# CNR-STIIMA-IRAS/rosdyn

Measured on NVIDIA B200. Metric: 6-DOF regressor+torque samples/sec (fp64), higher is better.
Workload: dtype f64

## Files before the change

### rosdyn_b200/csrc/gram_common.cuh

```cuda
#pragma once
#ifndef __CUDACC_RTC__
#include <cuda_runtime.h>
#endif

#include "chain_dev.h"
#include "spatial.cuh"

namespace rdb
{

#ifndef GF_TSPLIT
#define GF_TSPLIT 2
#endif
#ifndef GF_ZCOL
#define GF_ZCOL 1
#endif
constexpr int GF_KSPLIT = 4;
constexpr int GF_TS = GF_TSPLIT;
constexpr int GF_MMA_WARPS = GF_KSPLIT * GF_TS;
constexpr int GF_MAX_SLOTS = 4;
constexpr int GF_BAR_REDUCE = 1;

__device__ __forceinline__ void bar_sync(int id, int count) { asm volatile("bar.sync %0, %1;" ::"r"(id), "r"(count) : "memory"); }
__device__ __forceinline__ void dmma884f(double& d0, double& d1, double a, double b)
{
  asm volatile("mma.sync.aligned.m8n8k4.row.col.f64.f64.f64.f64 {%0,%1}, {%2}, {%3}, {%0,%1};\n" : "+d"(d0), "+d"(d1) : "d"(a), "d"(b));
}
__device__ __forceinline__ uint32_t smem_u32(const void* p) { return (uint32_t)__cvta_generic_to_shared(p); }
__device__ __forceinline__ void mbar_init(uint64_t* b, int count)
{
  asm volatile("mbarrier.init.shared::cta.b64 [%0], %1;" ::"r"(smem_u32(b)), "r"(count) : "memory");
}
__device__ __forceinline__ void mbar_arrive(uint64_t* b)
{
  asm volatile("{\n .reg .b64 st;\n mbarrier.arrive.shared::cta.b64 st, [%0];\n}" ::"r"(smem_u32(b)) : "memory");
}
__device__ __forceinline__ void mbar_wait(uint64_t* b, uint32_t parity)
{
  asm volatile(
      "{\n .reg .pred p;\n"
      "W: mbarrier.try_wait.parity.shared::cta.b64 p, [%0], %1;\n"
      " @p bra D;\n bra W;\n"
      "D:\n}" ::"r"(smem_u32(b)),
      "r"(parity)
      : "memory");
}

template <int V>
struct ic
{
  static constexpr int value = V;
};
template <int B, int E, class F>
__device__ __forceinline__ void static_for(F&& f)
{
  if constexpr (B < E)
  {
    f(ic<B>{});
    static_for<B + 1, E>(f);
  }
}

constexpr int GX_COLS = 8;
#ifndef GF_TAU_TILE
#define GF_TAU_TILE 0
#endif
template <int NJ, int X = 0, int Z = 0>
struct GramGeom
{
  static constexpr int P = 10 * NJ;
  static constexpr int TC = Z == 2 && !GF_TAU_TILE ? 0 : 1;
  __host__ __device__ static constexpr int inblk(int p)
  {
    constexpr int zord[10] = {9, 1, 2, 8, 3, 4, 5, 6, 7, 0};
    return Z == 2 ? zord[p] : (Z == 1 ? (p == 0 ? 9 : p - 1) : p);
  }
  __host__ __device__ static constexpr int param_at(int q)
  {
    constexpr int zinv[10] = {9, 1, 2, 4, 5, 6, 7, 8, 3, 0};
    return Z == 2 ? zinv[q] : (Z == 1 ? (q == 9 ? 0 : q + 1) : q);
  }
  __host__ __device__ static constexpr int pos(int l, int p) { return TC + 10 * (NJ - 1 - l) + inblk(p); }
  __host__ __device__ static constexpr bool stored(int j, int l, int p)
  {
    if (j != l || Z == 0) return true;
    if (Z == 1) return p != 0;
    return l == 0 ? (p == 1 || p == 2 || p == 9) : (p != 0 && p != 3);
  }
  __host__ __device__ static constexpr int rowlen(int j)
  {
    return Z == 2 ? TC + 10 * (NJ - 1 - j) + (j == 0 ? 3 : 8) : 1 + 10 * (NJ - j) - Z;
  }
  static constexpr int NPOS = rowlen(0);
  __host__ __device__ static constexpr int col_of(int q) { return q < TC ? P : 10 * (NJ - 1 - (q - TC) / 10) + param_at((q - TC) % 10); }
  __host__ __device__ static constexpr bool has_pos(int c) { return c / 10 > 0 || stored(0, 0, c % 10); }
  static constexpr int T = (NPOS + 7) / 8;
  static constexpr int NT = T * (T + 1) / 2;
  static constexpr int NF = T + 1 - TC;
  static constexpr int PARTIAL = NT * 64 + (TC ? 0 : 8 * T + 1);
  static constexpr int KPW = 8 / GF_KSPLIT;
  static constexpr int NSTEPS = NJ * KPW;
  __host__ __device__ static constexpr int threads(int slots) { return 32 * (GF_MMA_WARPS + slots); }
  __host__ __device__ static constexpr int rowbase(int j)
  {
    int o = 0;
    for (int i = 0; i < j; i++) o += (rowlen(i) + (X ? GX_COLS : 0)) * 32;
    return o;
  }
  __host__ __device__ static constexpr int taubase(int j) { return TC ? rowbase(j) : rowbase(NJ) + 32 * j; }
  static constexpr int SLOT_DOUBLES = rowbase(NJ) + (TC ? 0 : 32 * NJ);
  __host__ __device__ static constexpr int tile(int I, int J) { return I * T - I * (I - 1) / 2 + (J - I); }
  __host__ __device__ static constexpr bool owns(int I, int ts, int par) { return ts == 1 || (I & 1) == par; }
  __host__ __device__ static constexpr int ntiles(int ts, int par)
  {
    int n = 0;
    for (int I = 0; I < T; I++)
      if (owns(I, ts, par)) n += T - I;
    return n > 0 ? n : 1;
  }
  __host__ __device__ static constexpr int local(int I, int J, int ts, int par)
  {
    int n = 0;
    for (int K = 0; K < I; K++)
      if (owns(K, ts, par)) n += T - K;
    return n + (J - I);
  }
  __host__ __device__ static constexpr int bown(int I, int ts, int par)
  {
    int n = 0;
    for (int K = 0; K < I; K++)
      if (owns(K, ts, par)) n++;
    return n;
  }
  __host__ __device__ static constexpr int nbacc(int ts, int par) { return TC || (par != 0 && bown(T, ts, par) == 0) ? 1 : bown(T, ts, par) + (par == 0 ? 1 : 0); }
  __host__ __device__ static constexpr int tj(int j) { return (rowlen(j) + 7) / 8; }
  __host__ __device__ static constexpr int xtile(int j, int I)
  {
    int n = 0;
    for (int k = 0; k < j; k++) n += tj(k) + 1;
    return n + I;
  }
  __host__ __device__ static constexpr int nxt()
  {
    int n = 0;
    for (int k = 0; k < NJ; k++) n += tj(k) + 1;
    return n;
  }
  static constexpr int NXT = nxt();
  __host__ __device__ static constexpr bool xowns(int j, int I, int ts, int par) { return ts == 1 || ((I == tj(j) ? j : I) & 1) == par; }
  __host__ __device__ static constexpr int xlocal(int j, int I, int ts, int par)
  {
    int n = 0;
    for (int k = 0; k <= j; k++)
      for (int K = 0; K <= tj(k); K++)
      {
        if (k == j && K == I) return n;
        if (xowns(k, K, ts, par)) n++;
      }
    return n;
  }
  __host__ __device__ static constexpr int nxtiles(int ts, int par)
  {
    int n = 0;
    for (int k = 0; k < NJ; k++)
      for (int K = 0; K <= tj(k); K++)
        if (xowns(k, K, ts, par)) n++;
    return n;
  }
};

enum : int
{
  GXK_SAT = 1,
  GXK_OMEGA = 2,
  GXK_SGN = 3,
  GXK_SQ = 4,
  GXK_Q = 5,
  GXK_ONE = 6
};
struct GramComps
{
  int32_t ncols[8];
  int32_t kind[8][GX_COLS];
  double thr[8][GX_COLS], vmax[8][GX_COLS];
  double ithr[8][GX_COLS];
};

struct RtModel
{
  static constexpr bool RUNTIME = true;
};
enum : int
{
  MK_A = 0,
  MK_T = 1,
  MK_PI = 2,
  MK_G = 3
};
struct Zr
{
};
template <int S>
struct Un
{
};
template <class T>
struct tv_unit
{
  static constexpr int s = 0;
};
template <int S>
struct tv_unit<Un<S>>
{
  static constexpr int s = S;
};
template <class T>
struct tv_zero
{
  static constexpr bool v = false;
};
template <>
struct tv_zero<Zr>
{
  static constexpr bool v = true;
};

template <class M, int F, int L, int K, int NJ>
__device__ __forceinline__ auto kc(const ChainDev<NJ>& C)
{
  if constexpr (M::RUNTIME)
  {
    if constexpr (F == MK_A) return C.joint[L].A[K];
    else if constexpr (F == MK_T) return C.joint[L].t[K];
    else if constexpr (F == MK_PI) return C.link[L].pi[K];
    else return C.g[K];
  }
  else
  {
    constexpr double v = M::val(F, L, K);
    if constexpr (v == 0.0) return Zr{};
    else if constexpr (v == 1.0) return Un<1>{};
    else if constexpr (v == -1.0) return Un<-1>{};
    else return v;
  }
}

template <class A>
__device__ __forceinline__ double tv_d(A a)
{
  if constexpr (tv_zero<A>::v) return 0.0;
  else if constexpr (tv_unit<A>::s != 0) return (double)tv_unit<A>::s;
  else return a;
}
template <class A>
__device__ __forceinline__ auto tneg(A a)
{
  if constexpr (tv_zero<A>::v) return Zr{};
  else if constexpr (tv_unit<A>::s != 0) return Un<-tv_unit<A>::s>{};
  else return -a;
}
template <class A, class B>
__device__ __forceinline__ auto tmul(A a, B b)
{
  constexpr int ua = tv_unit<A>::s, ub = tv_unit<B>::s;
  if constexpr (tv_zero<A>::v || tv_zero<B>::v) return Zr{};
  else if constexpr (ua != 0 && ub != 0) return Un<ua * ub>{};
  else if constexpr (ua != 0) return ua > 0 ? b : -b;
  else if constexpr (ub != 0) return ub > 0 ? a : -a;
  else return __dmul_rn(a, b);
}
template <class A, class B>
__device__ __forceinline__ auto tadd(A a, B b)
{
  if constexpr (tv_zero<A>::v) return b;
  else if constexpr (tv_zero<B>::v) return a;
  else return __dadd_rn(tv_d(a), tv_d(b));
}
template <class A, class B, class C>
__device__ __forceinline__ auto tfma(A a, B b, C c)
{
  using P = decltype(tmul(a, b));
  if constexpr (tv_zero<P>::v) return c;
  else if constexpr (tv_zero<C>::v) return tmul(a, b);
  else if constexpr (tv_unit<A>::s != 0 || tv_unit<B>::s != 0) return tadd(tmul(a, b), c);
  else return __fma_rn(a, b, tv_d(c));
}

template <class X, class Y, class W>
struct T3
{
  X x;
  Y y;
  W z;
};
template <class X, class Y, class W>
__device__ __forceinline__ T3<X, Y, W> mk3(X x, Y y, W z)
{
  return T3<X, Y, W>{x, y, z};
}
template <class A>
__device__ __forceinline__ V3 tod3(const A& a)
{
  return V3{tv_d(a.x), tv_d(a.y), tv_d(a.z)};
}
template <class A, class B>
__device__ __forceinline__ auto tdot(const A& a, const B& b)
{
  return tfma(a.x, b.x, tfma(a.y, b.y, tmul(a.z, b.z)));
}
template <class A, class B>
__device__ __forceinline__ auto tcross(const A& a, const B& b)
{
  return mk3(tfma(a.y, b.z, tneg(tmul(a.z, b.y))), tfma(a.z, b.x, tneg(tmul(a.x, b.z))), tfma(a.x, b.y, tneg(tmul(a.y, b.x))));
}
template <class Cv, class A, class B>
__device__ __forceinline__ auto tcross_add(const Cv& c, const A& a, const B& b)
{
  return mk3(tfma(a.y, b.z, tfma(tneg(a.z), b.y, c.x)), tfma(a.z, b.x, tfma(tneg(a.x), b.z, c.y)), tfma(a.x, b.y, tfma(tneg(a.y), b.x, c.z)));
}
template <class R, class A>
__device__ __forceinline__ auto trotT(const R& r, const A& a)
{
  return mk3(tfma(r.x.x, a.x, tfma(r.y.x, a.y, tmul(r.z.x, a.z))), tfma(r.x.y, a.x, tfma(r.y.y, a.y, tmul(r.z.y, a.z))),
             tfma(r.x.z, a.x, tfma(r.y.z, a.y, tmul(r.z.z, a.z))));
}

template <int NJ>
struct GenIn
{
  double q[NJ], dq[NJ], ddq[NJ], sv[NJ], cv[NJ];
};
template <int NJ>
__device__ __forceinline__ void gen_load(const ChainDev<NJ>& C, const SamplesDev& in, int64_t i, GenIn<NJ>& x)
{
#pragma unroll
  for (int l = 0; l < NJ; l++)
  {
    x.q[l] = ld_in(in.q, C.joint[l].in, in.ld, i);
    x.dq[l] = ld_in(in.dq, C.joint[l].in, in.ld, i);
    x.ddq[l] = ld_in(in.ddq, C.joint[l].in, in.ld, i);
  }
}

template <int NJ>
__device__ __forceinline__ void gram_component_columns(const ChainDev<NJ>& C, const GramComps& comps, const SamplesDev& in, int64_t i,
                                                       double* __restrict__ slot, int lane)
{
  using G = GramGeom<NJ, 1>;
  double qv[NJ], dqv[NJ];
#pragma unroll
  for (int j = 0; j < NJ; j++)
  {
    qv[j] = ld_in(in.q, C.joint[j].in, in.ld, i);
    dqv[j] = ld_in(in.dq, C.joint[j].in, in.ld, i);
  }
  static_for<0, NJ>([&](auto jc) {
    constexpr int j = decltype(jc)::value;
    const double q = qv[j], dq = dqv[j];
    const int nc = comps.ncols[j];
    double* o = slot + G::rowbase(j) + G::rowlen(j) * 32;
#pragma unroll 1
    for (int c = 0; c < GX_COLS; c++)
    {
      double val = 0.0;
      if (c < nc)
      {
        const int kd = comps.kind[j][c];
        const double th = comps.thr[j][c], vm = comps.vmax[j][c];
        const double omega = fmin(fmax(dq, -vm), vm);
        if (kd == GXK_OMEGA) val = omega;
        else if (kd == GXK_Q) val = q;
        else if (kd == GXK_ONE) val = 1.0;
        else
        {
          const double r = omega * comps.ithr[j][c];
          if (kd == GXK_SAT) val = fmin(fmax(r, -1.0), 1.0);
          else
          {
            const double sg = omega == 0.0 ? 0.0 : (omega > th ? 1.0 : (omega < -th ? -1.0 : r));
            val = kd == GXK_SGN ? sg : omega * omega * sg;
          }
        }
      }
      o[c * 32 + (lane ^ (4 * (c & 3)))] = val;
    }
  });
}

template <bool GLOBAL>
__device__ __forceinline__ void st_row(double* p, double v)
{
  if (GLOBAL) __stcg(p, v);
  else *p = v;
}

template <class M, int NJ, int X, int Z, bool GLOBAL, int L, int J, bool OWN, class E0, class E1, class E2, class E3, class E4, class E5, class E6,
          class E7, class E8, class E9>
__device__ __forceinline__ void gram_emit(const ChainDev<NJ>& C, double (&tau)[NJ], double* __restrict__ slot, int lane, E0 e0, E1 e1, E2 e2, E3 e3,
                                          E4 e4, E5 e5, E6 e6, E7 e7, E8 e8, E9 e9)
{
  using G = GramGeom<NJ, X, Z>;
  auto P = [&](auto pc) { return kc<M, MK_PI, L, decltype(pc)::value>(C); };
  auto t0a = [&] {
    if constexpr (J == L && M::RUNTIME) return 0.0;
    else if constexpr (J == L) return Zr{};
    else return tau[J];
  }();
  const auto t0 = tfma(e8, P(ic<8>{}), tfma(e6, P(ic<6>{}), tfma(e4, P(ic<4>{}), tfma(e2, P(ic<2>{}), tfma(e0, P(ic<0>{}), t0a)))));
  const auto t1 = tfma(e9, P(ic<9>{}), tfma(e7, P(ic<7>{}), tfma(e5, P(ic<5>{}), tfma(e3, P(ic<3>{}), tmul(e1, P(ic<1>{}))))));
  tau[J] = tv_d(tadd(t0, t1));
  double* o = slot + G::rowbase(J);
  const double e[10] = {tv_d(e0), tv_d(e1), tv_d(e2), tv_d(e3), tv_d(e4), tv_d(e5), tv_d(e6), tv_d(e7), tv_d(e8), tv_d(e9)};
#pragma unroll
  for (int p = 0; p < 10; p++)
    if (G::stored(J, L, p))
      st_row<GLOBAL>(o + G::pos(L, p) * 32 + (lane ^ (4 * (G::pos(L, p) & 3))), e[p]);
}
template <class M, int NJ, int X, int Z, bool GLOBAL, int L, int J, class U, class S>
__device__ __forceinline__ void gram_project(const ChainDev<NJ>& C, double (&tau)[NJ], double* __restrict__ slot, int lane, const U& u, const S& s,
                                             const V3& fm, const V3& w, const V3& al)
{
  const auto h = tcross_add(tcross_add(tcross(u, al), w, tcross(w, u)), fm, s);
  const auto rho = tcross(s, w);
  gram_emit<M, NJ, X, Z, GLOBAL, L, J, false>(
      C, tau, slot, lane, tdot(u, fm), h.x, h.y, h.z, tfma(s.x, al.x, tmul(rho.x, w.x)),
      tfma(s.x, al.y, tfma(s.y, al.x, tfma(rho.x, w.y, tmul(rho.y, w.x)))), tfma(s.x, al.z, tfma(s.z, al.x, tfma(rho.x, w.z, tmul(rho.z, w.x)))),
      tfma(s.y, al.y, tmul(rho.y, w.y)), tfma(s.y, al.z, tfma(s.z, al.y, tfma(rho.y, w.z, tmul(rho.z, w.y)))), tfma(s.z, al.z, tmul(rho.z, w.z)));
}

template <int NJ, class M, int X, int Z, bool GLOBAL, bool LAZY>
__device__ __forceinline__ void gram_walk_rev(const ChainDev<NJ>& C, const GenIn<NJ>& x, const SamplesDev& in, double* __restrict__ slot, int64_t i,
                                              int lane, double (&tau)[NJ])
{
  static_assert(REV_AXIS[0] == 0.0 && REV_AXIS[1] == 0.0 && REV_AXIS[2] == 1.0, "the REV walk below is written for the axis s = e_z");
  V3 U[NJ], S[NJ];
  V3 v = v3(0, 0, 0), w = v3(0, 0, 0), a = v3(0, 0, 0), al = v3(0, 0, 0), g;
  static_for<0, NJ>([&](auto lc) {
    constexpr int l = decltype(lc)::value;
    const JointDev& J = C.joint[l];
    const double dql = LAZY ? ld_in(in.dq, J.in, in.ld, i) : x.dq[l], ddql = LAZY ? ld_in(in.ddq, J.in, in.ld, i) : x.ddq[l];
    const double sl = x.sv[l], cl = x.cv[l];
    const auto t = mk3(kc<M, MK_T, l, 0>(C), kc<M, MK_T, l, 1>(C), kc<M, MK_T, l, 2>(C));
    auto row = [&](auto kc_) {
      constexpr int k = decltype(kc_)::value;
      const auto a0 = kc<M, MK_A, l, 3 * k>(C);
      const auto a1 = kc<M, MK_A, l, 3 * k + 1>(C);
      return mk3(tfma(sl, a1, tmul(cl, a0)), tfma(-sl, a0, tmul(cl, a1)), kc<M, MK_A, l, 3 * k + 2>(C));
    };
    const auto R = mk3(row(ic<0>{}), row(ic<1>{}), row(ic<2>{}));
    v = tod3(trotT(R, tcross_add(v, w, t)));
    w = tod3(trotT(R, w));
    a = tod3(trotT(R, tcross_add(a, al, t)));
    al = tod3(trotT(R, al));
    if constexpr (l == 0) g = tod3(trotT(R, mk3(kc<M, MK_G, 0, 0>(C), kc<M, MK_G, 0, 1>(C), kc<M, MK_G, 0, 2>(C))));
    else g = tod3(trotT(R, g));
    w.z += dql;
    a.x = fma(v.y, dql, a.x);
    a.y = fma(-v.x, dql, a.y);
    al.x = fma(w.y, dql, al.x);
    al.y = fma(-w.x, dql, al.y);
    al.z += ddql;
    static_for<0, (l > 0 ? l - 1 : 0)>([&](auto jc) {
      constexpr int j = decltype(jc)::value;
      U[j] = tod3(trotT(R, tcross_add(U[j], S[j], t)));
      S[j] = tod3(trotT(R, S[j]));
    });
    const auto S1 = R.z;
    const auto U1 = mk3(tfma(t.x, R.y.x, tneg(tmul(t.y, R.x.x))), tfma(t.x, R.y.y, tneg(tmul(t.y, R.x.y))), tfma(t.x, R.y.z, tneg(tmul(t.y, R.x.z))));
    if constexpr (l > 0)
    {
      S[l - 1] = tod3(S1);
      U[l - 1] = tod3(U1);
    }
    const V3 fm = cross_add(a - g, w, v);
    static_for<0, l + 1>([&](auto jc) {
      constexpr int j = decltype(jc)::value;
      if constexpr (j == l)
      {
        const double e7 = w.x * w.y;
        gram_emit<M, NJ, X, Z, GLOBAL, l, j, true>(C, tau, slot, lane, Zr{}, fm.y, -fm.x, Zr{}, -e7, fma(w.x, w.x, -(w.y * w.y)),
                                                   fma(-w.y, w.z, al.x), e7, fma(w.x, w.z, al.y), al.z);
      }
      else if constexpr (j == l - 1) gram_project<M, NJ, X, Z, GLOBAL, l, j>(C, tau, slot, lane, U1, S1, fm, w, al);
      else gram_project<M, NJ, X, Z, GLOBAL, l, j>(C, tau, slot, lane, U[j], S[j], fm, w, al);
    });
  });
}

template <int NJ, int X, int Z, bool GLOBAL, bool LAZY>
__device__ __forceinline__ void gram_walk_gen(const ChainDev<NJ>& C, const GenIn<NJ>& x, const SamplesDev& in, double* __restrict__ slot, int64_t i,
                                              int lane, double (&tau)[NJ])
{
  using G = GramGeom<NJ, X, Z>;
  V3 U[NJ], S[NJ];
  V3 v = v3(0, 0, 0), w = v3(0, 0, 0), a = v3(0, 0, 0), al = v3(0, 0, 0);
  V3 g = v3(C.g);
#pragma unroll
  for (int l = 0; l < NJ; l++)
  {
    const JointDev& J = C.joint[l];
    const double dql = LAZY ? ld_in(in.dq, J.in, in.ld, i) : x.dq[l], ddql = LAZY ? ld_in(in.ddq, J.in, in.ld, i) : x.ddq[l];
    double R[9];
    const V3 t = J.type != RDB_JOINT_PRISMATIC ? v3(J.t) : axpy(v3(J.t), v3(J.axp), x.q[l]);
    if (J.type == RDB_JOINT_REVOLUTE)
    {
      const double c1 = 1.0 - x.cv[l];
#pragma unroll
      for (int k = 0; k < 9; k++) R[k] = fma(c1, J.C[k], fma(x.sv[l], J.B[k], J.A[k]));
    }
    else
    {
#pragma unroll
      for (int k = 0; k < 9; k++) R[k] = J.A[k];
    }
    v = rotT(R, cross_add(v, w, t));
    w = rotT(R, w);
    a = rotT(R, cross_add(a, al, t));
    al = rotT(R, al);
    g = rotT(R, g);
    const V3 axj = v3(J.ax);
    const V3 su = J.type == RDB_JOINT_PRISMATIC ? axj : v3(0, 0, 0);
    const V3 ss = J.type == RDB_JOINT_REVOLUTE ? axj : v3(0, 0, 0);
    v = axpy(v, su, dql);
    w = axpy(w, ss, dql);
    const V3 xl = cross_add(cross(w, su), v, ss);
    const V3 xa = cross(w, ss);
    a = axpy(axpy(a, xl, dql), su, ddql);
    al = axpy(axpy(al, xa, dql), ss, ddql);
    U[l] = su;
    S[l] = ss;
#pragma unroll
    for (int j = 0; j < l; j++)
    {
      U[j] = rotT(R, cross_add(U[j], S[j], t));
      S[j] = rotT(R, S[j]);
    }
    tau[l] = 0.0;
    const double* Pl = C.link[l].pi;
    const V3 fm = cross_add(a - g, w, v);
#pragma unroll
    for (int j = 0; j <= l; j++)
    {
      const V3 u = U[j], s = S[j];
      const V3 h = cross_add(cross_add(cross(u, al), w, cross(w, u)), fm, s);
      const V3 rho = cross(s, w);
      double e[10];
      e[0] = dot(u, fm);
      e[1] = h.x;
      e[2] = h.y;
      e[3] = h.z;
      e[4] = fma(s.x, al.x, rho.x * w.x);
      e[5] = fma(s.x, al.y, fma(s.y, al.x, fma(rho.x, w.y, rho.y * w.x)));
      e[6] = fma(s.x, al.z, fma(s.z, al.x, fma(rho.x, w.z, rho.z * w.x)));
      e[7] = fma(s.y, al.y, rho.y * w.y);
      e[8] = fma(s.y, al.z, fma(s.z, al.y, fma(rho.y, w.z, rho.z * w.y)));
      e[9] = fma(s.z, al.z, rho.z * w.z);
      double t0 = tau[j], t1 = e[1] * Pl[1];
#pragma unroll
      for (int p = 0; p < 10; p += 2) t0 = fma(e[p], Pl[p], t0);
#pragma unroll
      for (int p = 3; p < 10; p += 2) t1 = fma(e[p], Pl[p], t1);
      tau[j] = t0 + t1;
      double* o = slot + G::rowbase(j);
#pragma unroll
      for (int p = 0; p < 10; p++) st_row<GLOBAL>(o + G::pos(l, p) * 32 + (lane ^ (4 * (G::pos(l, p) & 3))), e[p]);
    }
  }
}

template <int NJ, bool REV, int X, int Z = 0, bool GLOBAL = false, bool LAZY = false, class M = RtModel>
__device__ __forceinline__ void gram_generate(const ChainDev<NJ>& C, const GramComps* comps, const GenIn<NJ>& x, const SamplesDev& in,
                                              const double* __restrict__ tau_meas, double* __restrict__ slot, int64_t i, int lane)
{
  static_assert(!Z || REV, "the zero mass column of a link on its own joint exists for revolute joints only");
  static_assert(REV || M::RUNTIME, "compile-time models are built for the REV walk");
  using G = GramGeom<NJ, X, Z>;
  double tau[NJ];
  if constexpr (REV) gram_walk_rev<NJ, M, X, Z, GLOBAL, LAZY>(C, x, in, slot, i, lane, tau);
  else gram_walk_gen<NJ, X, Z, GLOBAL, LAZY>(C, x, in, slot, i, lane, tau);
#pragma unroll
  for (int j = 0; j < NJ; j++)
  {
    const double tv = tau_meas ? __ldcs(tau_meas + (int64_t)C.joint[j].in * in.ld + i) : tau[j];
    st_row<GLOBAL>(slot + G::taubase(j) + lane, tv);
  }
  if (X) gram_component_columns<NJ>(C, *comps, in, i, slot, lane);
}

template <int NJ, int X, int Z = 0, bool GLOBAL = false>
__device__ __noinline__ void gram_zero_lane(double* __restrict__ slot, int lane)
{
  using G = GramGeom<NJ, X, Z>;
  for (int j = 0; j < NJ; j++)
  {
    for (int c = 0; c < G::rowlen(j); c++) st_row<GLOBAL>(slot + G::rowbase(j) + c * 32 + (lane ^ (4 * (c & 3))), 0.0);
    if (!G::TC) st_row<GLOBAL>(slot + G::taubase(j) + lane, 0.0);
    if (X)
      for (int c = 0; c < GX_COLS; c++) st_row<GLOBAL>(slot + G::rowbase(j) + (G::rowlen(j) + c) * 32 + (lane ^ (4 * (c & 3))), 0.0);
  }
}

}
```

### rosdyn_b200/csrc/gram_fused.cuh

```cuda
#pragma once
#include "gram_common.cuh"

namespace rdb
{

template <int NJ, int J, int X = 0, int Z = 0>
__device__ __forceinline__ void gram_load_frags(const double* __restrict__ slot, int kk, int lane, double (&b)[GramGeom<NJ, 0, Z>::NF])
{
  using G = GramGeom<NJ, X, Z>;
  constexpr int T = G::T, L = G::rowlen(J), TJ = G::tj(J);
  const int g = lane >> 2, t = lane & 3;
  const double* rowp = slot + G::rowbase(J) + ((4 * kk + t) ^ (4 * (g & 3)));
#pragma unroll
  for (int I = 0; I < T; I++)
  {
    if (I >= TJ) continue;
    const int col = 8 * I + g;
    if (8 * I + 7 < L || col < L) b[I] = rowp[col * 32];
    else b[I] = 0.0;
  }
  if constexpr (!G::TC) b[T] = slot[G::taubase(J) + 4 * kk + t];
}
template <int NJ, int PAR, int J, int Z>
__device__ __forceinline__ void gram_mma_step(const double (&b)[GramGeom<NJ, 0, Z>::NF], double (&acc)[GramGeom<NJ, 0, Z>::ntiles(GF_TS, PAR)][2])
{
  using G = GramGeom<NJ, 0, Z>;
  constexpr int T = G::T, TJ = G::tj(J);
#pragma unroll
  for (int I = 0; I < T; I++)
  {
    if (I >= TJ || !G::owns(I, GF_TS, PAR)) continue;
#pragma unroll
    for (int K = I; K < T; K++)
      if (K < TJ) dmma884f(acc[G::local(I, K, GF_TS, PAR)][0], acc[G::local(I, K, GF_TS, PAR)][1], b[I], b[K]);
  }
}
template <int NJ, int PAR, int J, int Z>
__device__ __forceinline__ void gram_tau_step(const double (&b)[GramGeom<NJ, 0, Z>::NF], double (&bacc)[GramGeom<NJ, 0, Z>::nbacc(GF_TS, PAR)])
{
  using G = GramGeom<NJ, 0, Z>;
  if constexpr (!G::TC)
  {
    static_for<0, G::tj(J)>([&](auto Ic) {
      constexpr int I = decltype(Ic)::value;
      if constexpr (G::owns(I, GF_TS, PAR)) bacc[G::bown(I, GF_TS, PAR)] = fma(b[I], b[G::T], bacc[G::bown(I, GF_TS, PAR)]);
    });
    if constexpr (PAR == 0) bacc[G::nbacc(GF_TS, PAR) - 1] = fma(b[G::T], b[G::T], bacc[G::nbacc(GF_TS, PAR) - 1]);
  }
}
template <int NJ, int PAR, int STEP, int Z>
__device__ __forceinline__ void gram_consume_steps(const double* __restrict__ slot, int ks, int lane, const double (&bcur)[GramGeom<NJ, 0, Z>::NF],
                                                   double (&acc)[GramGeom<NJ, 0, Z>::ntiles(GF_TS, PAR)][2],
                                                   double (&bacc)[GramGeom<NJ, 0, Z>::nbacc(GF_TS, PAR)])
{
  using G = GramGeom<NJ, 0, Z>;
  constexpr int J = STEP / G::KPW;
  if constexpr (STEP + 1 < G::NSTEPS)
  {
    double bnext[G::NF];
    gram_load_frags<NJ, (STEP + 1) / G::KPW, 0, Z>(slot, ks * G::KPW + (STEP + 1) % G::KPW, lane, bnext);
    gram_mma_step<NJ, PAR, J, Z>(bcur, acc);
    gram_tau_step<NJ, PAR, J, Z>(bcur, bacc);
    gram_consume_steps<NJ, PAR, STEP + 1, Z>(slot, ks, lane, bnext, acc, bacc);
  }
  else
  {
    gram_mma_step<NJ, PAR, J, Z>(bcur, acc);
    gram_tau_step<NJ, PAR, J, Z>(bcur, bacc);
  }
}
template <int NJ, int PAR, int Z>
__device__ __forceinline__ void gram_consume_slot(const double* __restrict__ slot, int ks, int lane,
                                                  double (&acc)[GramGeom<NJ, 0, Z>::ntiles(GF_TS, PAR)][2],
                                                  double (&bacc)[GramGeom<NJ, 0, Z>::nbacc(GF_TS, PAR)])
{
  using G = GramGeom<NJ, 0, Z>;
  double b0[G::NF];
  gram_load_frags<NJ, 0, 0, Z>(slot, ks * G::KPW, lane, b0);
  gram_consume_steps<NJ, PAR, 0, Z>(slot, ks, lane, b0, acc, bacc);
}

#ifndef GF_SPIN_NS
#define GF_SPIN_NS 32
#endif
struct GramBars
{
  uint64_t full[GF_MAX_SLOTS], empty[GF_MAX_SLOTS];
  uint32_t filled[GF_MAX_SLOTS];
  uint32_t drained[GF_MAX_SLOTS];
};
__device__ __forceinline__ uint32_t ld_acquire_u32(const uint32_t* p)
{
  uint32_t v;
  asm volatile("ld.acquire.cta.shared.u32 %0, [%1];" : "=r"(v) : "r"(smem_u32(p)) : "memory");
  return v;
}
__device__ __forceinline__ void st_release_u32(uint32_t* p, uint32_t v)
{
  asm volatile("st.release.cta.shared.u32 [%0], %1;" ::"r"(smem_u32(p)), "r"(v) : "memory");
}
__device__ __forceinline__ void red_release_inc(uint32_t* p)
{
  asm volatile("red.release.cta.shared.add.u32 [%0], 1;" ::"r"(smem_u32(p)) : "memory");
}
__device__ __forceinline__ void wait_counter_ge(const uint32_t* p, uint32_t v)
{
  while (ld_acquire_u32(p) < v) __nanosleep(GF_SPIN_NS);
}

template <int NJ, int PAR, int Z>
__device__ __forceinline__ void gram_mma_reduce(double (&acc)[GramGeom<NJ, 0, Z>::ntiles(GF_TS, PAR)][2], double* smem, int ks, int lane)
{
  using G = GramGeom<NJ, 0, Z>;
  bar_sync(GF_BAR_REDUCE, 32 * GF_MMA_WARPS);
  const int g = lane >> 2, t = lane & 3;
  for (int w = 0; w < GF_KSPLIT; w++)
  {
    if (ks == w)
    {
#pragma unroll
      for (int I = 0; I < G::T; I++)
      {
        if (!G::owns(I, GF_TS, PAR)) continue;
#pragma unroll
        for (int J = I; J < G::T; J++)
        {
          double* o = smem + G::tile(I, J) * 64 + g * 8 + 2 * t;
          const int k = G::local(I, J, GF_TS, PAR);
          if (w == 0)
          {
            o[0] = acc[k][0];
            o[1] = acc[k][1];
          }
          else
          {
            o[0] += acc[k][0];
            o[1] += acc[k][1];
          }
        }
      }
    }
    bar_sync(GF_BAR_REDUCE, 32 * GF_MMA_WARPS);
  }
}
template <int NJ, int PAR, int Z>
__device__ __forceinline__ void gram_tau_reduce(double (&bacc)[GramGeom<NJ, 0, Z>::nbacc(GF_TS, PAR)], double* smem, int ks, int lane)
{
  using G = GramGeom<NJ, 0, Z>;
  if constexpr (!G::TC)
  {
    constexpr int NB = G::nbacc(GF_TS, PAR);
#pragma unroll
    for (int k = 0; k < NB; k++)
    {
      bacc[k] += __shfl_xor_sync(0xffffffffu, bacc[k], 1);
      bacc[k] += __shfl_xor_sync(0xffffffffu, bacc[k], 2);
    }
    const int g = lane >> 2, t = lane & 3;
    double* ob = smem + G::NT * 64;
    for (int w = 0; w < GF_KSPLIT; w++)
    {
      if (ks == w && t == 0)
      {
#pragma unroll
        for (int I = 0; I < G::T; I++)
        {
          if (!G::owns(I, GF_TS, PAR)) continue;
          double& o = ob[8 * I + g];
          o = w == 0 ? bacc[G::bown(I, GF_TS, PAR)] : o + bacc[G::bown(I, GF_TS, PAR)];
        }
        if (PAR == 0 && g == 0) ob[8 * G::T] = w == 0 ? bacc[NB - 1] : ob[8 * G::T] + bacc[NB - 1];
      }
      bar_sync(GF_BAR_REDUCE, 32 * GF_MMA_WARPS);
    }
  }
}

template <int NJ, int SLOTS, int PAR, int Z>
__device__ __forceinline__ void gram_mma_role(const SamplesDev& in, double* smem, GramBars* bars, int ks, int lane, int dbg)
{
  using G = GramGeom<NJ, 0, Z>;
  constexpr int NTP = G::ntiles(GF_TS, PAR);
  double acc[NTP][2], bacc[G::nbacc(GF_TS, PAR)];
#pragma unroll
  for (int k = 0; k < NTP; k++) acc[k][0] = acc[k][1] = 0.0;
#pragma unroll
  for (int k = 0; k < G::nbacc(GF_TS, PAR); k++) bacc[k] = 0.0;
  const int64_t ngroups = (in.n + 31) / 32;
  const int64_t stride = (int64_t)gridDim.x * SLOTS;
  uint32_t parity = 0;
  for (int64_t base = (int64_t)blockIdx.x * SLOTS; base < ngroups; base += stride, parity ^= 1)
  {
#pragma unroll 1
    for (int s = 0; s < SLOTS; s++)
    {
      if (base + s >= ngroups) break;
      const double* slot = smem + (size_t)s * G::SLOT_DOUBLES;
      mbar_wait(&bars->full[s], parity);
      if (!(dbg & 2))
      {
        gram_consume_slot<NJ, PAR, Z>(slot, ks, lane, acc, bacc);
      }
      if (base + s + stride < ngroups)
      {
        __syncwarp();
        if (lane == 0) mbar_arrive(&bars->empty[s]);
      }
    }
  }
  gram_mma_reduce<NJ, PAR, Z>(acc, smem, ks, lane);
  gram_tau_reduce<NJ, PAR, Z>(bacc, smem, ks, lane);
}

template <int NJ, int J>
__device__ __forceinline__ double gram_load_xfrag(const double* __restrict__ slot, int kk, int lane)
{
  using G = GramGeom<NJ, 1>;
  const int g = lane >> 2, t = lane & 3;
  return slot[G::rowbase(J) + (G::rowlen(J) + g) * 32 + ((4 * kk + t) ^ (4 * (g & 3)))];
}
template <int NJ, int PAR, int J, int Z = 0>
__device__ __forceinline__ void gram_cross_step(const double (&b)[GramGeom<NJ, 0, Z>::NF], double bx,
                                                double (&acc)[GramGeom<NJ, 1, Z>::nxtiles(GF_TS, PAR)][2])
{
  using G = GramGeom<NJ, 1, Z>;
  static_for<0, G::tj(J) + 1>([&](auto Ic) {
    constexpr int I = decltype(Ic)::value;
    if constexpr (G::xowns(J, I, GF_TS, PAR))
    {
      constexpr int k = G::xlocal(J, I, GF_TS, PAR);
      if constexpr (I < G::tj(J)) dmma884f(acc[k][0], acc[k][1], b[I], bx);
      else dmma884f(acc[k][0], acc[k][1], bx, bx);
    }
  });
}
template <int NJ, int PAR, int Z = 0>
__device__ __forceinline__ void gram_cross_reduce_smem(double (&acc)[GramGeom<NJ, 1, Z>::nxtiles(GF_TS, PAR)][2], double* smem, int ks, int lane)
{
  using G = GramGeom<NJ, 1, Z>;
  bar_sync(GF_BAR_REDUCE, 32 * GF_MMA_WARPS);
  const int g = lane >> 2, t = lane & 3;
  for (int w = 0; w < GF_KSPLIT; w++)
  {
    if (ks == w)
    {
      static_for<0, NJ>([&](auto jc) {
        constexpr int j = decltype(jc)::value;
        static_for<0, G::tj(j) + 1>([&](auto Ic) {
          constexpr int I = decltype(Ic)::value;
          if constexpr (G::xowns(j, I, GF_TS, PAR))
          {
            double* o = smem + G::xtile(j, I) * 64 + g * 8 + 2 * t;
            constexpr int k = G::xlocal(j, I, GF_TS, PAR);
            if (w == 0)
            {
              o[0] = acc[k][0];
              o[1] = acc[k][1];
            }
            else
            {
              o[0] += acc[k][0];
              o[1] += acc[k][1];
            }
          }
        });
      });
    }
    bar_sync(GF_BAR_REDUCE, 32 * GF_MMA_WARPS);
  }
}

template <int NJ, int SLOTS, bool REV, int X, int Z, class M>
__device__ __forceinline__ void gram_gen_role(const ChainDev<NJ>& C, const GramComps& comps, const SamplesDev& in,
                                              const double* __restrict__ tau_meas, double* smem, GramBars* bars, int s, int lane, int dbg)
{
  using G = GramGeom<NJ, X, Z>;
  double* slot = smem + (size_t)s * G::SLOT_DOUBLES;
  const int64_t ngroups = (in.n + 31) / 32;
  const int64_t stride = (int64_t)gridDim.x * SLOTS;
  uint32_t parity = 1;
  for (int64_t grp = (int64_t)blockIdx.x * SLOTS + s; grp < ngroups; grp += stride, parity ^= 1)
  {
    const int64_t i = grp * 32 + lane;
    GenIn<NJ> cur;
    gen_load<NJ>(C, in, min(i, in.n - 1), cur);
    trig_all<NJ>(cur.q, cur.sv, cur.cv);
    mbar_wait(&bars->empty[s], parity);
    if (!(dbg & 1))
    {
      gram_generate<NJ, REV, X, Z, false, false, M>(C, &comps, cur, in, tau_meas, slot, min(i, in.n - 1), lane);
      if (i >= in.n) gram_zero_lane<NJ, X, Z>(slot, lane);
    }
    __syncwarp();
    if (lane == 0) mbar_arrive(&bars->full[s]);
  }
}

template <int NJ, int SLOTS, int GENS, bool REV, int Z, class M>
__device__ __forceinline__ void gram_gen_role_c(const ChainDev<NJ>& C, const SamplesDev& in, const double* __restrict__ tau_meas, double* smem,
                                                GramBars* bars, int w, int lane, int dbg)
{
  using G = GramGeom<NJ, 0, Z>;
  const int64_t ngroups = (in.n + 31) / 32;
  const int64_t nk = ngroups > blockIdx.x ? (ngroups - blockIdx.x + gridDim.x - 1) / gridDim.x : 0;
  for (int64_t k = w; k < nk; k += GENS)
  {
    const int s = (int)(k % SLOTS);
    const uint32_t u = (uint32_t)(k / SLOTS);
    const int64_t i = ((int64_t)blockIdx.x + k * gridDim.x) * 32 + lane;
    GenIn<NJ> cur;
    gen_load<NJ>(C, in, min(i, in.n - 1), cur);
    trig_all<NJ>(cur.q, cur.sv, cur.cv);
    wait_counter_ge(&bars->drained[s], GF_MMA_WARPS * u);
    double* slot = smem + (size_t)s * G::SLOT_DOUBLES;
    if (!(dbg & 1))
    {
      gram_generate<NJ, REV, 0, Z, false, false, M>(C, nullptr, cur, in, tau_meas, slot, min(i, in.n - 1), lane);
      if (i >= in.n) gram_zero_lane<NJ, 0, Z>(slot, lane);
    }
    __syncwarp();
    if (lane == 0) st_release_u32(&bars->filled[s], u + 1);
  }
}

template <int NJ, int SLOTS, int PAR, int Z>
__device__ __forceinline__ void gram_mma_role_c(const SamplesDev& in, double* smem, GramBars* bars, int ks, int lane, int dbg)
{
  using G = GramGeom<NJ, 0, Z>;
  constexpr int NTP = G::ntiles(GF_TS, PAR);
  double acc[NTP][2], bacc[G::nbacc(GF_TS, PAR)];
#pragma unroll
  for (int k = 0; k < NTP; k++) acc[k][0] = acc[k][1] = 0.0;
#pragma unroll
  for (int k = 0; k < G::nbacc(GF_TS, PAR); k++) bacc[k] = 0.0;
  const int64_t ngroups = (in.n + 31) / 32;
  const int64_t nk = ngroups > blockIdx.x ? (ngroups - blockIdx.x + gridDim.x - 1) / gridDim.x : 0;
#pragma unroll 1
  for (int64_t k = 0; k < nk; k++)
  {
    const int s = (int)(k % SLOTS);
    const uint32_t u = (uint32_t)(k / SLOTS);
    const double* slot = smem + (size_t)s * G::SLOT_DOUBLES;
    wait_counter_ge(&bars->filled[s], u + 1);
    if (!(dbg & 2))
    {
      gram_consume_slot<NJ, PAR, Z>(slot, ks, lane, acc, bacc);
    }
    __syncwarp();
    if (lane == 0) red_release_inc(&bars->drained[s]);
  }
  gram_mma_reduce<NJ, PAR, Z>(acc, smem, ks, lane);
  gram_tau_reduce<NJ, PAR, Z>(bacc, smem, ks, lane);
}

template <int NJ, int XC>
__host__ __device__ constexpr int gram_ext_side_doubles()
{
  return NJ * XC * 32;
}
template <int NJ, int XC>
__device__ __forceinline__ void gram_component_park(const GenIn<NJ>& x, double* __restrict__ side, int lane)
{
  static_assert(XC >= 2, "q and Dq of a joint are staged in its first two columns");
#pragma unroll
  for (int j = 0; j < NJ; j++)
  {
    side[(j * XC) * 32 + lane] = x.dq[j];
    side[(j * XC + 1) * 32 + lane] = x.q[j];
  }
}
template <int NJ, int XC>
__device__ __forceinline__ void gram_component_side(const GramComps& comps, double* __restrict__ side, int lane)
{
#pragma unroll 1
  for (int j = 0; j < NJ; j++)
  {
    double* o = side + (j * XC) * 32 + lane;
    const double dq = o[0], q = o[32];
    const int nc = comps.ncols[j];
#pragma unroll(XC <= 4 ? XC : 1)
    for (int c = 0; c < XC; c++)
    {
      double val = 0.0;
      if (c < nc)
      {
        const int kd = comps.kind[j][c];
        const double th = comps.thr[j][c], vm = comps.vmax[j][c];
        const double omega = fmin(fmax(dq, -vm), vm);
        if (kd == GXK_OMEGA) val = omega;
        else if (kd == GXK_Q) val = q;
        else if (kd == GXK_ONE) val = 1.0;
        else
        {
          const double r = omega * comps.ithr[j][c];
          if (kd == GXK_SAT) val = fmin(fmax(r, -1.0), 1.0);
          else
          {
            const double sg = omega == 0.0 ? 0.0 : (omega > th ? 1.0 : (omega < -th ? -1.0 : r));
            val = kd == GXK_SGN ? sg : omega * omega * sg;
          }
        }
      }
      o[c * 32] = val;
    }
  }
}
template <int J, int XC>
__device__ __forceinline__ double gram_load_xside(const double* __restrict__ side, int kk, int lane)
{
  const int g = lane >> 2, t = lane & 3;
  return g < XC ? side[(J * XC + g) * 32 + 4 * kk + t] : 0.0;
}
template <int NJ, int PAR, int STEP, int Z, int XC>
__device__ __forceinline__ void gram_ext_steps(const double* __restrict__ slot, const double* __restrict__ side, int ks, int lane,
                                               const double (&bcur)[GramGeom<NJ, 0, Z>::NF], double bxcur,
                                               double (&acc)[GramGeom<NJ, 0, Z>::ntiles(GF_TS, PAR)][2],
                                               double (&xacc)[GramGeom<NJ, 1, Z>::nxtiles(GF_TS, PAR)][2])
{
  using G = GramGeom<NJ, 0, Z>;
  constexpr int J = STEP / G::KPW;
  if constexpr (STEP + 1 < G::NSTEPS)
  {
    double bnext[G::NF];
    constexpr int JN = (STEP + 1) / G::KPW;
    const int kn = ks * G::KPW + (STEP + 1) % G::KPW;
    gram_load_frags<NJ, JN, 0, Z>(slot, kn, lane, bnext);
    const double bxn = gram_load_xside<JN, XC>(side, kn, lane);
    gram_mma_step<NJ, PAR, J, Z>(bcur, acc);
    gram_cross_step<NJ, PAR, J, Z>(bcur, bxcur, xacc);
    gram_ext_steps<NJ, PAR, STEP + 1, Z, XC>(slot, side, ks, lane, bnext, bxn, acc, xacc);
  }
  else
  {
    gram_mma_step<NJ, PAR, J, Z>(bcur, acc);
    gram_cross_step<NJ, PAR, J, Z>(bcur, bxcur, xacc);
  }
}

template <int NJ, int SLOTS, int PAR, int Z, int XC>
__device__ __forceinline__ void gram_ext_mma_role(const SamplesDev& in, double* smem, const double* side0, GramBars* bars, int ks, int lane)
{
  using G0 = GramGeom<NJ, 0, Z>;
  using GX = GramGeom<NJ, 1, Z>;
  double acc[G0::ntiles(GF_TS, PAR)][2], xacc[GX::nxtiles(GF_TS, PAR)][2];
#pragma unroll
  for (int k = 0; k < G0::ntiles(GF_TS, PAR); k++) acc[k][0] = acc[k][1] = 0.0;
#pragma unroll
  for (int k = 0; k < GX::nxtiles(GF_TS, PAR); k++) xacc[k][0] = xacc[k][1] = 0.0;
  const int64_t ngroups = (in.n + 31) / 32;
  const int64_t nk = ngroups > blockIdx.x ? (ngroups - blockIdx.x + gridDim.x - 1) / gridDim.x : 0;
#pragma unroll 1
  for (int64_t k = 0; k < nk; k++)
  {
    const int s = (int)(k % SLOTS);
    const uint32_t u = (uint32_t)(k / SLOTS);
    const double* slot = smem + (size_t)s * G0::SLOT_DOUBLES;
    const double* side = side0 + (size_t)s * gram_ext_side_doubles<NJ, XC>();
    wait_counter_ge(&bars->filled[s], u + 1);
    double b0[G0::NF];
    gram_load_frags<NJ, 0, 0, Z>(slot, ks * G0::KPW, lane, b0);
    const double bx0 = gram_load_xside<0, XC>(side, ks * G0::KPW, lane);
    gram_ext_steps<NJ, PAR, 0, Z, XC>(slot, side, ks, lane, b0, bx0, acc, xacc);
    __syncwarp();
    if (lane == 0) red_release_inc(&bars->drained[s]);
  }
  gram_mma_reduce<NJ, PAR, Z>(acc, smem, ks, lane);
  gram_cross_reduce_smem<NJ, PAR, Z>(xacc, smem + G0::NT * 64, ks, lane);
}

template <int NJ, int SLOTS, int GENS, bool REV, int XC, class M = RtModel>
__global__ void __launch_bounds__(GramGeom<NJ>::threads(GENS), 1)
    gram_ext_kernel(const __grid_constant__ ChainDev<NJ> C, const __grid_constant__ GramComps comps, const SamplesDev in,
                    const double* __restrict__ tau_meas, double* __restrict__ partial)
{
  constexpr int Z = GF_ZCOL && REV ? 1 : 0;
  using G0 = GramGeom<NJ, 0, Z>;
  using GX = GramGeom<NJ, 1, Z>;
  constexpr int NOUT = (G0::NT + GX::NXT) * 64;
  constexpr int SIDE = gram_ext_side_doubles<NJ, XC>();
  extern __shared__ __align__(16) double smem[];
  __shared__ GramBars bars;
  double* const side0 = smem + (G0::SLOT_DOUBLES * SLOTS > NOUT ? G0::SLOT_DOUBLES * SLOTS : NOUT);
  const int warp = threadIdx.x >> 5, lane = threadIdx.x & 31;
  if (threadIdx.x < SLOTS)
  {
    bars.filled[threadIdx.x] = 0;
    bars.drained[threadIdx.x] = 0;
  }
  __syncthreads();
  if (warp >= GF_MMA_WARPS)
  {
    const int w = warp - GF_MMA_WARPS;
    const int64_t ngroups = (in.n + 31) / 32;
    const int64_t nk = ngroups > blockIdx.x ? (ngroups - blockIdx.x + gridDim.x - 1) / gridDim.x : 0;
    for (int64_t k = w; k < nk; k += GENS)
    {
      const int s = (int)(k % SLOTS);
      const uint32_t u = (uint32_t)(k / SLOTS);
      const int64_t i = ((int64_t)blockIdx.x + k * gridDim.x) * 32 + lane;
      GenIn<NJ> cur;
      gen_load<NJ>(C, in, min(i, in.n - 1), cur);
      trig_all<NJ>(cur.q, cur.sv, cur.cv);
      wait_counter_ge(&bars.drained[s], GF_MMA_WARPS * u);
      double* slot = smem + (size_t)s * G0::SLOT_DOUBLES;
      double* side = side0 + (size_t)s * SIDE;
      gram_component_park<NJ, XC>(cur, side, lane);
      gram_generate<NJ, REV, 0, Z, false, false, M>(C, nullptr, cur, in, tau_meas, slot, min(i, in.n - 1), lane);
      gram_component_side<NJ, XC>(comps, side, lane);
      if (i >= in.n)
      {
        gram_zero_lane<NJ, 0, Z>(slot, lane);
        for (int c = 0; c < NJ * XC; c++) side[c * 32 + lane] = 0.0;
      }
      __syncwarp();
      if (lane == 0) st_release_u32(&bars.filled[s], u + 1);
    }
    return;
  }
  const int mma_id = warp, ks = mma_id % GF_KSPLIT;
  if (GF_TS == 1 || mma_id < GF_KSPLIT) gram_ext_mma_role<NJ, SLOTS, 0, Z, XC>(in, smem, side0, &bars, ks, lane);
  else gram_ext_mma_role<NJ, SLOTS, 1, Z, XC>(in, smem, side0, &bars, ks, lane);
  double* out = partial + (size_t)blockIdx.x * NOUT;
  for (int k = mma_id * 32 + lane; k < NOUT; k += 32 * GF_MMA_WARPS) out[k] = smem[k];
}

template <int NJ, int SLOTS, bool REV, int X, int GENS = SLOTS, class M = RtModel>
__global__ void __launch_bounds__(GramGeom<NJ>::threads(GENS), 1)
    gram_fused_kernel(const __grid_constant__ ChainDev<NJ> C, const __grid_constant__ GramComps comps, const SamplesDev in,
                      const double* __restrict__ tau_meas, double* __restrict__ partial, const int dbg)
{
  constexpr int Z = GF_ZCOL && REV && X == 0 ? 2 : 0;
  using G = GramGeom<NJ, X, Z>;
  extern __shared__ __align__(16) double smem[];
  __shared__ GramBars bars;
  const int warp = threadIdx.x >> 5, lane = threadIdx.x & 31;
  if (threadIdx.x == 0)
  {
    for (int s = 0; s < SLOTS; s++)
    {
      mbar_init(&bars.full[s], 1);
      mbar_init(&bars.empty[s], GF_MMA_WARPS);
      bars.filled[s] = 0;
      bars.drained[s] = 0;
    }
    asm volatile("fence.mbarrier_init.release.cluster;" ::: "memory");
  }
  __syncthreads();
  if (warp >= GF_MMA_WARPS)
  {
    if constexpr (GENS != SLOTS) gram_gen_role_c<NJ, SLOTS, GENS, REV, Z, M>(C, in, tau_meas, smem, &bars, warp - GF_MMA_WARPS, lane, dbg);
    else gram_gen_role<NJ, SLOTS, REV, X, Z, M>(C, comps, in, tau_meas, smem, &bars, warp - GF_MMA_WARPS, lane, dbg);
    return;
  }
  const int mma_id = warp;
  const int ks = mma_id % GF_KSPLIT;
  constexpr int NOUT = X ? G::NXT * 64 : G::PARTIAL;
  static_assert(X == 0, "the extended model runs through gram_ext_kernel");
  {
    if constexpr (GENS != SLOTS)
    {
      if (GF_TS == 1 || mma_id < GF_KSPLIT) gram_mma_role_c<NJ, SLOTS, 0, Z>(in, smem, &bars, ks, lane, dbg);
      else gram_mma_role_c<NJ, SLOTS, 1, Z>(in, smem, &bars, ks, lane, dbg);
    }
    else
    {
      if (GF_TS == 1 || mma_id < GF_KSPLIT) gram_mma_role<NJ, SLOTS, 0, Z>(in, smem, &bars, ks, lane, dbg);
      else gram_mma_role<NJ, SLOTS, 1, Z>(in, smem, &bars, ks, lane, dbg);
    }
  }
  double* out = partial + (size_t)blockIdx.x * NOUT;
  for (int k = mma_id * 32 + lane; k < NOUT; k += 32 * GF_MMA_WARPS) out[k] = smem[k];
}

}
```

Baseline: 2.285 billion.

## Prefetch next slot fragments across slot boundary and balance tile ownership

The MMA consumer warps now release the current slot, wait for the next slot and load its first fragments before issuing the last step's DMMAs. This hides shared-memory load latency across slot boundaries instead of stalling at the start of each slot. Separately, for Z==2 the split of tile rows between the two parity warps is chosen greedily by DMMA count rather than by row parity, aiming to balance work. The release now happens before the last step's MMAs run, which is safe only because the operands are already in registers, and the prefetch adds register pressure.

```diff
diff --git a/rosdyn_b200/csrc/gram_common.cuh b/rosdyn_b200/csrc/gram_common.cuh
--- a/rosdyn_b200/csrc/gram_common.cuh
+++ b/rosdyn_b200/csrc/gram_common.cuh
@@ -110,7 +110,27 @@
   __host__ __device__ static constexpr int taubase(int j) { return TC ? rowbase(j) : rowbase(NJ) + 32 * j; }
   static constexpr int SLOT_DOUBLES = rowbase(NJ) + (TC ? 0 : 32 * NJ);
   __host__ __device__ static constexpr int tile(int I, int J) { return I * T - I * (I - 1) / 2 + (J - I); }
-  __host__ __device__ static constexpr bool owns(int I, int ts, int par) { return ts == 1 || (I & 1) == par; }
+  __host__ __device__ static constexpr int tj(int j) { return (rowlen(j) + 7) / 8; }
+  __host__ __device__ static constexpr int row_dmma(int I)
+  {
+    int n = 0;
+    for (int j = 0; j < NJ; j++) n += tj(j) > I ? tj(j) - I : 0;
+    return n;
+  }
+  __host__ __device__ static constexpr unsigned own_mask()
+  {
+    unsigned m = 0;
+    int n0 = 0, n1 = 0;
+    for (int I = 0; I < T; I++)
+    {
+      const bool one = Z == 2 ? n1 < n0 : (I & 1) != 0;
+      (one ? n1 : n0) += row_dmma(I);
+      if (one) m |= 1u << I;
+    }
+    return m;
+  }
+  static constexpr unsigned OWN1 = own_mask();
+  __host__ __device__ static constexpr bool owns(int I, int ts, int par) { return ts == 1 || (int)((OWN1 >> I) & 1u) == par; }
   __host__ __device__ static constexpr int ntiles(int ts, int par)
   {
     int n = 0;
@@ -133,7 +153,6 @@
     return n;
   }
   __host__ __device__ static constexpr int nbacc(int ts, int par) { return TC || (par != 0 && bown(T, ts, par) == 0) ? 1 : bown(T, ts, par) + (par == 0 ? 1 : 0); }
-  __host__ __device__ static constexpr int tj(int j) { return (rowlen(j) + 7) / 8; }
   __host__ __device__ static constexpr int xtile(int j, int I)
   {
     int n = 0;
diff --git a/rosdyn_b200/csrc/gram_fused.cuh b/rosdyn_b200/csrc/gram_fused.cuh
--- a/rosdyn_b200/csrc/gram_fused.cuh
+++ b/rosdyn_b200/csrc/gram_fused.cuh
@@ -48,10 +48,10 @@
     if constexpr (PAR == 0) bacc[G::nbacc(GF_TS, PAR) - 1] = fma(b[G::T], b[G::T], bacc[G::nbacc(GF_TS, PAR) - 1]);
   }
 }
-template <int NJ, int PAR, int STEP, int Z>
+template <int NJ, int PAR, int STEP, int Z, class Next>
 __device__ __forceinline__ void gram_consume_steps(const double* __restrict__ slot, int ks, int lane, const double (&bcur)[GramGeom<NJ, 0, Z>::NF],
                                                    double (&acc)[GramGeom<NJ, 0, Z>::ntiles(GF_TS, PAR)][2],
-                                                   double (&bacc)[GramGeom<NJ, 0, Z>::nbacc(GF_TS, PAR)])
+                                                   double (&bacc)[GramGeom<NJ, 0, Z>::nbacc(GF_TS, PAR)], Next&& next)
 {
   using G = GramGeom<NJ, 0, Z>;
   constexpr int J = STEP / G::KPW;
@@ -61,25 +61,15 @@
     gram_load_frags<NJ, (STEP + 1) / G::KPW, 0, Z>(slot, ks * G::KPW + (STEP + 1) % G::KPW, lane, bnext);
     gram_mma_step<NJ, PAR, J, Z>(bcur, acc);
     gram_tau_step<NJ, PAR, J, Z>(bcur, bacc);
-    gram_consume_steps<NJ, PAR, STEP + 1, Z>(slot, ks, lane, bnext, acc, bacc);
+    gram_consume_steps<NJ, PAR, STEP + 1, Z>(slot, ks, lane, bnext, acc, bacc, next);
   }
   else
   {
+    next();
     gram_mma_step<NJ, PAR, J, Z>(bcur, acc);
     gram_tau_step<NJ, PAR, J, Z>(bcur, bacc);
   }
 }
-template <int NJ, int PAR, int Z>
-__device__ __forceinline__ void gram_consume_slot(const double* __restrict__ slot, int ks, int lane,
-                                                  double (&acc)[GramGeom<NJ, 0, Z>::ntiles(GF_TS, PAR)][2],
-                                                  double (&bacc)[GramGeom<NJ, 0, Z>::nbacc(GF_TS, PAR)])
-{
-  using G = GramGeom<NJ, 0, Z>;
-  double b0[G::NF];
-  gram_load_frags<NJ, 0, 0, Z>(slot, ks * G::KPW, lane, b0);
-  gram_consume_steps<NJ, PAR, 0, Z>(slot, ks, lane, b0, acc, bacc);
-}
-
 #ifndef GF_SPIN_NS
 #define GF_SPIN_NS 32
 #endif
@@ -187,26 +177,29 @@
 #pragma unroll
   for (int k = 0; k < G::nbacc(GF_TS, PAR); k++) bacc[k] = 0.0;
   const int64_t ngroups = (in.n + 31) / 32;
-  const int64_t stride = (int64_t)gridDim.x * SLOTS;
-  uint32_t parity = 0;
-  for (int64_t base = (int64_t)blockIdx.x * SLOTS; base < ngroups; base += stride, parity ^= 1)
-  {
+  auto grp = [&](int64_t k) { return ((int64_t)blockIdx.x + k / SLOTS * gridDim.x) * SLOTS + k % SLOTS; };
+  double b0[G::NF];
+  if (grp(0) < ngroups)
+  {
+    mbar_wait(&bars->full[0], 0);
+    gram_load_frags<NJ, 0, 0, Z>(smem, ks * G::KPW, lane, b0);
+  }
 #pragma unroll 1
-    for (int s = 0; s < SLOTS; s++)
-    {
-      if (base + s >= ngroups) break;
-      const double* slot = smem + (size_t)s * G::SLOT_DOUBLES;
-      mbar_wait(&bars->full[s], parity);
-      if (!(dbg & 2))
+  for (int64_t k = 0; grp(k) < ngroups; k++)
+  {
+    const int s = (int)(k % SLOTS);
+    auto next = [&] {
+      __syncwarp();
+      if (lane == 0 && grp(k + SLOTS) < ngroups) mbar_arrive(&bars->empty[s]);
+      if (grp(k + 1) < ngroups)
       {
-        gram_consume_slot<NJ, PAR, Z>(slot, ks, lane, acc, bacc);
+        const int sn = (int)((k + 1) % SLOTS);
+        mbar_wait(&bars->full[sn], (uint32_t)((k + 1) / SLOTS) & 1);
+        gram_load_frags<NJ, 0, 0, Z>(smem + (size_t)sn * G::SLOT_DOUBLES, ks * G::KPW, lane, b0);
       }
-      if (base + s + stride < ngroups)
-      {
-        __syncwarp();
-        if (lane == 0) mbar_arrive(&bars->empty[s]);
-      }
-    }
+    };
+    if (!(dbg & 2)) gram_consume_steps<NJ, PAR, 0, Z>(smem + (size_t)s * G::SLOT_DOUBLES, ks, lane, b0, acc, bacc, next);
+    else next();
   }
   gram_mma_reduce<NJ, PAR, Z>(acc, smem, ks, lane);
   gram_tau_reduce<NJ, PAR, Z>(bacc, smem, ks, lane);
@@ -335,19 +328,28 @@
   for (int k = 0; k < G::nbacc(GF_TS, PAR); k++) bacc[k] = 0.0;
   const int64_t ngroups = (in.n + 31) / 32;
   const int64_t nk = ngroups > blockIdx.x ? (ngroups - blockIdx.x + gridDim.x - 1) / gridDim.x : 0;
+  double b0[G::NF];
+  if (nk > 0)
+  {
+    wait_counter_ge(&bars->filled[0], 1);
+    gram_load_frags<NJ, 0, 0, Z>(smem, ks * G::KPW, lane, b0);
+  }
 #pragma unroll 1
   for (int64_t k = 0; k < nk; k++)
   {
     const int s = (int)(k % SLOTS);
-    const uint32_t u = (uint32_t)(k / SLOTS);
-    const double* slot = smem + (size_t)s * G::SLOT_DOUBLES;
-    wait_counter_ge(&bars->filled[s], u + 1);
-    if (!(dbg & 2))
-    {
-      gram_consume_slot<NJ, PAR, Z>(slot, ks, lane, acc, bacc);
-    }
-    __syncwarp();
-    if (lane == 0) red_release_inc(&bars->drained[s]);
+    auto next = [&] {
+      __syncwarp();
+      if (lane == 0) red_release_inc(&bars->drained[s]);
+      if (k + 1 < nk)
+      {
+        const int sn = (int)((k + 1) % SLOTS);
+        wait_counter_ge(&bars->filled[sn], (uint32_t)((k + 1) / SLOTS) + 1);
+        gram_load_frags<NJ, 0, 0, Z>(smem + (size_t)sn * G::SLOT_DOUBLES, ks * G::KPW, lane, b0);
+      }
+    };
+    if (!(dbg & 2)) gram_consume_steps<NJ, PAR, 0, Z>(smem + (size_t)s * G::SLOT_DOUBLES, ks, lane, b0, acc, bacc, next);
+    else next();
   }
   gram_mma_reduce<NJ, PAR, Z>(acc, smem, ks, lane);
   gram_tau_reduce<NJ, PAR, Z>(bacc, smem, ks, lane);
```

Result: slower. 2.248 billion (median of 6 runs) (-1.6%).
